# worxli/ORB_SLAM

Measured on AMD Instinct MI355X. Metric: frames/sec ORB extract+match (640x480, 1000 kp), higher is better.
Workload: dtype u8

## Files before the change

orb_slam_amd/csrc/orbx_device.h:

```cpp
#pragma once

#include <hip/hip_runtime.h>
#include <stdint.h>

#include "orbx_sincos.h"

namespace orbx {

#include "orbx_sincos_table.inc"

constexpr int kBlock = 256;
constexpr int kWaves = kBlock / 64;

__device__ inline float fast_atan2_deg(float y, float x)
{
    const float p1 = 0.9997878412794807f * (float)(180 / M_PI);
    const float p3 = -0.3258083974640975f * (float)(180 / M_PI);
    const float p5 = 0.1555786518463281f * (float)(180 / M_PI);
    const float p7 = -0.04432655554792128f * (float)(180 / M_PI);
    const float eps = (float)2.220446049250313e-16;
    const float ax = fabsf(x), ay = fabsf(y);
    float a;
    if (ax >= ay) {
        const float c = __fdiv_rn(ay, __fadd_rn(ax, eps));
// ... 356 lines not shown
            if (cl == m + 1) s.vars[0] = x;
            if (cl == 1) s.vars[2] = x;
        }
        if (k >= P) {
            if (cr <= m) posR[cr - 1] = x;
            if (cr == m) s.vars[1] = x;
            cr--;
        }
    }
    __syncthreads();
    for (int k = tid; k < m; k += kBlock) {
        const int i = posL[k], j = posR[k];
        const uint32_t t = a[i];
        a[i] = a[j];
        a[j] = t;
    }
    const int cut = (m == 0) ? s.vars[2] : min(s.vars[0], s.vars[1]);
    __syncthreads();
    return cut;
}

__device__ inline int floor_log2(int n)
{
    return 31 - __clz(n);
}

__device__ inline void block_nth_element(uint32_t* a, int n, int nth, int* pos, BlockScratch& s, int pivot_mode = 0)
{
    if (n == 0 || nth == n) return;
    int first = 0, last = n;
    int depth = 2 * floor_log2(n);
    while (last - first > 3) {
        if (depth == 0) {
            if (threadIdx.x == 0) {
                heap_select(a + first, nth + 1 - first, last - first);
                const uint32_t t = a[first];
                a[first] = a[nth];
                a[nth] = t;
            }
            __syncthreads();
            return;
        }
        --depth;
        if (threadIdx.x == 0) nth_pivot_step(a, first, last, pivot_mode);
        __syncthreads();
        const int cut = block_hoare_partition(a, first, last, pos, s);
        if (cut <= nth) first = cut;
        else last = cut;
    }
    if (threadIdx.x == 0) insertion_sort(a, first, last);
    __syncthreads();
}

__device__ inline void lds_wave_sync()
{
    __builtin_amdgcn_fence(__ATOMIC_RELEASE, "wavefront");
    __builtin_amdgcn_wave_barrier();
    __builtin_amdgcn_fence(__ATOMIC_ACQUIRE, "wavefront");
}

__device__ inline void global_wave_sync()
{
    __builtin_amdgcn_fence(__ATOMIC_RELEASE, "workgroup");
    __builtin_amdgcn_wave_barrier();
    __builtin_amdgcn_fence(__ATOMIC_ACQUIRE, "workgroup");
}

template <bool kGlobal>
__device__ inline void nth_sync()
{
    if constexpr (kGlobal) global_wave_sync();
    else lds_wave_sync();
}

__device__ inline int wave_min_int(int v)
{
#pragma unroll
    for (int o = 32; o > 0; o >>= 1) v = min(v, __shfl_xor(v, o, 64));
    return v;
}

template <bool kGlobal = false, typename E>
__device__ inline int wave_hoare_partition(E* a, int lo, int hi, int* pos)
{
    int* posR = pos;
    int* posL = pos + (hi - lo) / 2 + 1;
    const int lane = threadIdx.x & 63;
    const uint32_t P = kp_key(a[lo]);
    const int len = hi - lo - 1;
    const int chunk = (len + 63) / 64;
    const int s0 = min(lo + 1 + lane * chunk, hi), s1 = min(s0 + chunk, hi);
    int nle = 0, nge = 0;
    for (int x = s0; x < s1; x++) {
        const uint32_t k = kp_key(a[x]);
        nle += (k <= P);
        nge += (k >= P);
    }
    int le_incl, ge_incl;
    if (len < 65536) {
        const int both = wave_inclusive_scan(nle | (nge << 16));
        le_incl = both & 0xFFFF;
        ge_incl = (int)((uint32_t)both >> 16);
    } else {
        le_incl = wave_inclusive_scan(nle);
        ge_incl = wave_inclusive_scan(nge);
    }
    const int tot_ge = __builtin_amdgcn_readlane(ge_incl, 63);
    const int le_before = le_incl - nle;
    const int ge_after_chunk = tot_ge - ge_incl;
    int cl = le_before, cr = ge_after_chunk + nge, best = 0;
    for (int x = s0; x < s1; x++) {
        best = max(best, min(cl, cr));
        const uint32_t k = kp_key(a[x]);
        cl += (k <= P);
        cr -= (k >= P);
    }
    best = max(best, min(cl, cr));
    const int m = wave_max(best);
    int lm1 = 0x7fffffff, rm = -1, l1 = 0x7fffffff;
    cl = le_before;
    cr = ge_after_chunk + nge;
    for (int x = s0; x < s1; x++) {
        const uint32_t k = kp_key(a[x]);
        if (k <= P) {
            cl++;
            if (cl <= m) posL[cl - 1] = x;
            if (cl == m + 1) lm1 = x;
            if (cl == 1) l1 = x;
        }
        if (k >= P) {
            if (cr <= m) posR[cr - 1] = x;
            if (cr == m) rm = x;
            cr--;
        }
    }
    auto from_lane = [](int v, bool have, int none) {
        const unsigned long long b = __ballot(have);
        return b ? __builtin_amdgcn_readlane(v, (int)__builtin_ctzll(b)) : none;
    };
    lm1 = from_lane(lm1, lm1 != 0x7fffffff, 0x7fffffff);
    l1 = from_lane(l1, l1 != 0x7fffffff, 0x7fffffff);
    rm = from_lane(rm, rm >= 0, -1);
    nth_sync<kGlobal>();
    for (int k = lane; k < m; k += 64) {
        const int i = posL[k], j = posR[k];
        const E t = a[i];
        a[i] = a[j];
        a[j] = t;
    }
    nth_sync<kGlobal>();
    return (m == 0) ? l1 : min(lm1, rm);
}

template <bool kGlobal = false, typename E>
__device__ inline void wave_nth_element(E* a, int n, int nth, int* pos, int pivot_mode = 0)
{
    if (n == 0 || nth == n) return;
    const int lane = threadIdx.x & 63;
    int first = 0, last = n;
    int depth = 2 * floor_log2(n);
    while (last - first > 3) {
        if (depth == 0) {
            if (lane == 0) {
                heap_select(a + first, nth + 1 - first, last - first);
                const E t = a[first];
                a[first] = a[nth];
                a[nth] = t;
            }
            nth_sync<kGlobal>();
            return;
        }
        --depth;
        if (lane == 0) nth_pivot_step(a, first, last, pivot_mode);
        nth_sync<kGlobal>();
        const int cut = wave_hoare_partition<kGlobal>(a, first, last, pos);
        if (cut <= nth) first = cut;
        else last = cut;
    }
    if (lane == 0) insertion_sort(a, first, last);
    nth_sync<kGlobal>();
}

}
```

orb_slam_amd/csrc/orbx_extract.hip:

```cpp
#include <algorithm>
#include <type_traits>

#include "orbx_device.h"
#include "orbx_internal.h"

namespace orbx {

constexpr size_t kRetainLds = 128 * 1024;
constexpr int kRetainCellCap = 512;
constexpr int kSplitMinFrames = 16;
constexpr size_t kResizeLds = 96 * 1024;

__constant__ __attribute__((aligned(4))) int8_t c_pattern[256][4] = {
#include "orbx_pattern.inc"
};

#ifdef ORBX_FAST_PROFILE
__device__ unsigned long long g_fast_prof[24];
__device__ inline unsigned long long fp_stamp()
{
    unsigned long long t;
    asm volatile("s_memtime %0\n\ts_waitcnt lgkmcnt(0)" : "=s"(t)::"memory");
    return t;
}
// ... 1129 lines not shown
        tot[k] = 0;
        ret[k] = 0;
        nomore[k] = false;
        if (64 * k < nCells && c < nCells) {
            tot[k] = counts[c];
            if (a.cells[L.cell_base + c].valid) {
                if (tot[k] > nfc) {
                    ret[k] = nfc;
                } else {
                    ret[k] = tot[k];
                    toDist += nfc - tot[k];
                    nomore[k] = true;
                    nNoMore++;
                }
            }
        }
    }
    toDist = wave_sum(toDist);
    nNoMore = wave_sum(nNoMore);
    while (toDist > 0 && nNoMore < nCells) {
        const int nNew = nfc + (int)ceilf(__fdiv_rn((float)toDist, (float)(nCells - nNoMore)));
        int td = 0, nm = 0;
#pragma unroll
        for (int k = 0; k < kPer; k++) {
            if (64 * k >= nCells) break;
            const int c = lane + 64 * k;
            if (c < nCells && !nomore[k]) {
                if (tot[k] > nNew) {
                    ret[k] = nNew;
                } else {
                    ret[k] = tot[k];
                    td += nNew - tot[k];
                    nomore[k] = true;
                    nm++;
                }
            }
        }
        toDist = wave_sum(td);
        nNoMore += wave_sum(nm);
    }
    int base = 0, my_keep = 0, my_pre = 0;
#pragma unroll
    for (int k = 0; k < kPer; k++) {
        if (64 * k >= nCells) break;
        const int c = lane + 64 * k;
        const int take = (c < nCells && tot[k] > 0 && ret[k] > 0) ? min(tot[k], ret[k]) : 0;
        const int incl = wave_inclusive_scan(take);
        const int kk = __builtin_amdgcn_readlane(ret[k], cell & 63), pp = __builtin_amdgcn_readlane(base + incl - take, cell & 63);
        if ((cell >> 6) == k) {
            my_keep = kk;
            my_pre = pp;
        }
        base += __builtin_amdgcn_readlane(incl, 63);
    }
    *keep_c = my_keep;
    *pre_c = my_pre;
    *level_total = base;
}

constexpr float kHarrisK = 0.04f;
constexpr float kHarrisScale = 1.0f / ((1 << 2) * 7 * 255.0f);
constexpr float kHarrisScale4 = kHarrisScale * kHarrisScale * kHarrisScale * kHarrisScale;

__global__ __launch_bounds__(256) void k_harris_cells(ExtractArgs a)
{
    const int cell = blockIdx.x, f = blockIdx.y;
    const CellGeom C = cget(a.cells, cell);
    if (!C.valid) return;
    const int n = min(a.cell_count[(size_t)f * a.ncells + cell], C.list_cap);
    const LevelGeom L = cget(a.levels, C.level);
    const LevelSrc ls = level_src(a, f, C.level, L.off, L.stride);
    const int stride = ls.stride;
    const uint8_t* img = ls.base + (size_t)kEdge * stride + kEdge;
    const uint32_t* src = a.cell_lists + (size_t)f * a.list_entries + C.list_off;
    uint64_t* dst = a.cell_keys64 + (size_t)f * a.list_entries + C.list_off;
    for (int i = threadIdx.x; i < n; i += blockDim.x) {
        const uint32_t e = src[i];
        const int y = (int)((e >> 12) & 0xFFF), x = (int)(e & 0xFFF);
        const uint8_t* p0 = img + (ptrdiff_t)(y - 4) * stride + (x - 4);
        int r0[9], r1[9], r2[9];
#pragma unroll
        for (int j = 0; j < 9; j++) {
            r0[j] = p0[j];
            r1[j] = p0[stride + j];
        }
        int sa = 0, sb = 0, sc = 0;
#pragma unroll
        for (int rr = 2; rr < 9; rr++) {
#pragma unroll
            for (int j = 0; j < 9; j++) r2[j] = p0[(ptrdiff_t)rr * stride + j];
#pragma unroll
            for (int j = 1; j < 8; j++) {
                const int Ix = (r1[j + 1] - r1[j - 1]) * 2 + (r0[j + 1] - r0[j - 1]) + (r2[j + 1] - r2[j - 1]);
                const int Iy = (r2[j] - r0[j]) * 2 + (r2[j - 1] - r0[j - 1]) + (r2[j + 1] - r0[j + 1]);
                sa += Ix * Ix;
                sb += Iy * Iy;
                sc += Ix * Iy;
            }
#pragma unroll
            for (int j = 0; j < 9; j++) {
                r0[j] = r1[j];
                r1[j] = r2[j];
            }
        }
        const float fa = (float)sa, fb = (float)sb, fc = (float)sc;
        const float s2 = __fadd_rn(fa, fb);
        const float t = a.fp_contract
                            ? __fmaf_rn(-__fmul_rn(kHarrisK, s2), s2, __fmaf_rn(fa, fb, -__fmul_rn(fc, fc)))
                            : __fsub_rn(__fsub_rn(__fmul_rn(fa, fb), __fmul_rn(fc, fc)),
                                        __fmul_rn(__fmul_rn(kHarrisK, s2), s2));
        const float resp = __fmul_rn(t, kHarrisScale4);
        dst[i] = (uint64_t)harris_key(resp) << 32 | (e & 0xFFFFFFu);
    }
}

template <typename E>
__device__ inline E* cell_entries(const ExtractArgs& a)
{
    if constexpr (sizeof(E) == 8) return a.cell_keys64;
    else return a.cell_lists;
}
template <typename E>
__device__ inline E* level_entries(const ExtractArgs& a)
{
    if constexpr (sizeof(E) == 8) return a.level_keys64;
    else return a.level_keys;
}

template <typename E>
__global__ __launch_bounds__(256) void k_retain_cells(ExtractArgs a, int waves_per_block, int wave_words)
{
    extern __shared__ __attribute__((aligned(16))) uint32_t sbuf[];
    const int wv = threadIdx.x >> 6, lane = threadIdx.x & 63;
    const int cell = blockIdx.x * waves_per_block + wv, f = blockIdx.y;
    if (cell >= a.ncells) return;
    E* list = reinterpret_cast<E*>(sbuf + (size_t)wv * wave_words);
    int* pos = reinterpret_cast<int*>(list + kRetainCellCap);
    const CellGeom C = cget(a.cells, cell);
    const LevelGeom L = cget(a.levels, C.level);
    const int c = cell - L.cell_base;
    const int32_t* counts = a.cell_count + (size_t)f * a.ncells + L.cell_base;
    int k, pre, level_total;
    level_quota(a, L, counts, c, &k, &pre, &level_total);
    if (c == 0 && lane == 0) a.level_count[(size_t)f * a.nlevels + C.level] = min(level_total, L.level_cap);
    if (level_total > L.level_cap) {
        if (lane == 0) atomicOr(a.error_flags, 2);
        return;
    }
    const int n = counts[c];
    if (n == 0 || k == 0) return;
    const int take = min(n, k);
    E* src = cell_entries<E>(a) + (size_t)f * a.list_entries + C.list_off;
    E* dst = level_entries<E>(a) + (size_t)f * a.level_entries + L.level_off + pre;
    if (n > k && n <= kRetainCellCap) {
        stage_to_lds<8>(list, n, lane, 64, [&](int i) { return src[i]; });
        lds_wave_sync();
        wave_nth_element(list, n, k, pos, a.nth_pivot);
        for (int i = lane; i < take; i += 64) dst[i] = list[i];
    } else if (n > k) {
        int* gpos = a.retain_scratch + (size_t)f * (a.list_entries + 4 * a.ncells) + C.list_off + 4 * cell;
        wave_nth_element<true>(src, n, k, gpos, a.nth_pivot);
        for (int i = lane; i < take; i += 64) dst[i] = src[i];
    } else {
        for (int i = lane; i < take; i += 64) dst[i] = src[i];
    }
}

template <typename E>
__global__ __launch_bounds__(256) void k_retain_levels(ExtractArgs a, int waves_per_block, int wave_words)
{
    extern __shared__ __attribute__((aligned(16))) uint32_t sbuf[];
    const int wv = threadIdx.x >> 6, lane = threadIdx.x & 63;
    const int level = blockIdx.x * waves_per_block + wv, f = blockIdx.y;
    if (level >= a.nlevels) return;
    const LevelGeom L = cget(a.levels, level);
    int32_t* cnt = a.level_count + (size_t)f * a.nlevels + level;
    const int nlev = *cnt;
    if (nlev <= L.n_desired) return;
    E* list = reinterpret_cast<E*>(sbuf + (size_t)wv * wave_words);
    int* pos = reinterpret_cast<int*>(list + a.max_level_cap);
    E* g = level_entries<E>(a) + (size_t)f * a.level_entries + L.level_off;
    stage_to_lds<8>(list, nlev, lane, 64, [&](int i) { return g[i]; });
    lds_wave_sync();
    wave_nth_element(list, nlev, L.n_desired, pos, a.nth_pivot);
    for (int i = lane; i < L.n_desired; i += 64) g[i] = list[i];
    if (lane == 0) *cnt = L.n_desired;
}

typedef float orbx_f2 __attribute__((ext_vector_type(2)));

__device__ __forceinline__ void blur_hrow(uint32_t wl, uint32_t wc, uint32_t wr, orbx_f2 (&o)[2])
{
    int hs[4];
    blur_hsum_w(wl, wc, wr, hs);
    o[0] = orbx_f2{(float)hs[0], (float)hs[1]};
    o[1] = orbx_f2{(float)hs[2], (float)hs[3]};
}

__device__ __forceinline__ uint32_t blur_vstep(const orbx_f2 (&R)[7][2], uint32_t raw, const bool (&inside)[4],
                                               const bool (&tail_col)[4], bool any_tail)
{
    constexpr float kInv = 1.0f / 65536.0f;
    constexpr float k0 = 55.0f * kInv, k1 = 49.0f * kInv, k2 = 34.0f * kInv, k3 = 18.0f * kInv;
    float sv[4];
#pragma unroll
    for (int h = 0; h < 2; h++) {
        orbx_f2 N = R[3][h] * k0;
        N = __builtin_elementwise_fma(R[2][h] + R[4][h], orbx_f2{k1, k1}, N);
        N = __builtin_elementwise_fma(R[1][h] + R[5][h], orbx_f2{k2, k2}, N);
        N = __builtin_elementwise_fma(R[0][h] + R[6][h], orbx_f2{k3, k3}, N);
        sv[2 * h] = N.x;
        sv[2 * h + 1] = N.y;
        if (any_tail) {
            const orbx_f2 tl2 = N + 0.5f;
            if (tail_col[2 * h]) sv[2 * h] = floorf(tl2.x);
            if (tail_col[2 * h + 1]) sv[2 * h + 1] = floorf(tl2.y);
        }
    }
    uint32_t word = raw;
#pragma unroll
    for (int j = 0; j < 4; j++)
        if (inside[j]) word = __builtin_amdgcn_cvt_pk_u8_f32(sv[j], j, word);
    return word;
}

__device__ __forceinline__ void blur_block(const ExtractArgs& a, const int4* tiles, const int bx, const int f)
{
    const int4 tl = cget(tiles, bx);
    const int wi = tl.y + (threadIdx.x >> 6), lane = threadIdx.x & 63;
    if (wi >= tl.z * tl.w) return;
    const LevelGeom L = cget(a.levels, tl.x);
    const int strip = wi / tl.z, chunk = wi - strip * tl.z;
    const int ndw = L.stride >> 2;
    const int dw = kBlurChunkCols * chunk - 1 + lane;
    const bool out = lane >= 1 && lane <= kBlurChunkCols && dw < ndw;
    const int x = 4 * min(max(dw, 0), ndw - 1);
    const int y0 = strip * kBlurStrip, y1 = min(y0 + kBlurStrip, L.ph);
    const uint8_t* src = a.pyr_raw + (size_t)f * a.frame_pyr_bytes + L.off;
    uint8_t* dst = a.pyr_blur + (size_t)f * a.frame_pyr_bytes + L.off;
    const uint32_t stride = (uint32_t)L.stride;
    auto ld = [&](int y) { return *reinterpret_cast<const uint32_t*>(src + ((uint32_t)y * stride + (uint32_t)x)); };
    auto st = [&](int y, uint32_t v) {
        if (out) *reinterpret_cast<uint32_t*>(dst + ((uint32_t)y * stride + (uint32_t)x)) = v;
    };
    auto left = [&](uint32_t v) { return (uint32_t)__builtin_amdgcn_update_dpp(0, (int)v, 0x138, 0xf, 0xf, false); };
    auto right = [&](uint32_t v) { return (uint32_t)__builtin_amdgcn_update_dpp(0, (int)v, 0x130, 0xf, 0xf, false); };
    const int iy0 = kEdge, iy1 = kEdge + L.h;
    const int ya = min(max(y0, iy0), y1), yb = max(min(y1, iy1), ya);
    uint32_t keep_mask = 0;
#pragma unroll
    for (int j = 0; j < 4; j++)
        if (x + j < L.pw) keep_mask |= 0xFFu << (8 * j);
    auto copy_rows = [&](int ylo, int yhi) {
        for (int yc = ylo; yc < yhi; yc += 4) {
            uint32_t v[4];
#pragma unroll
            for (int k = 0; k < 4; k++) v[k] = ld(min(yc + k, yhi - 1));
#pragma unroll
            for (int k = 0; k < 4; k++)
                if (yc + k < yhi) st(yc + k, v[k] & keep_mask);
        }
    };
    copy_rows(y0, ya);
    if (ya < yb) {
        int half_even[4];
        bool inside[4];
#pragma unroll
        for (int j = 0; j < 4; j++) {
            const int xi = x + j - kEdge;
            inside[j] = xi >= 0 && xi < L.w;
            half_even[j] = xi < L.nvec_blur;
        }
        bool tail_col[4], any_tail = false;
#pragma unroll
        for (int j = 0; j < 4; j++) {
            tail_col[j] = inside[j] && !half_even[j];
            any_tail = any_tail || tail_col[j];
        }
        orbx_f2 R[7][2];
        auto hrow = [&](uint32_t c, orbx_f2 (&o)[2]) { blur_hrow(left(c), c, right(c), o); };
        uint32_t C[3];
        {
            uint32_t w0[6];
#pragma unroll
            for (int k = 0; k < 6; k++) w0[k] = ld(ya - 3 + k);
#pragma unroll
            for (int k = 0; k < 6; k++) {
                hrow(w0[k], R[k]);
                if (k >= 3) C[k - 3] = w0[k];
            }
        }
        constexpr int kBlurChunk = 7;
        for (int yc = ya; yc < yb; yc += kBlurChunk) {
            uint32_t wc[kBlurChunk];
#pragma unroll
            for (int k = 0; k < kBlurChunk; k++) wc[k] = ld(min(yc + k, yb - 1) + 3);
#pragma unroll
            for (int k = 0; k < kBlurChunk; k++) {
                const int y = yc + k;
                hrow(wc[k], R[6]);
                const uint32_t word = blur_vstep(R, C[0], inside, tail_col, any_tail);
                if (y < yb) st(y, word & keep_mask);
#pragma unroll
                for (int kk = 0; kk < 6; kk++)
#pragma unroll
                    for (int h = 0; h < 2; h++) R[kk][h] = R[kk + 1][h];
                C[0] = C[1];
// ... 201 lines not shown
};

template <bool kFma>
__global__ __launch_bounds__(256) __attribute__((amdgpu_waves_per_eu(5))) void k_describe(ExtractArgs a, int nframes)
{
    __shared__ __attribute__((aligned(16))) uint8_t s_patch[2 * kWaves][kDescWaveBytes];
    __shared__ int2 s_mom[2 * kWaves];
    __shared__ DescTrig s_trig[2 * kWaves];
    const XcdBlock xb = xcd_block();
    const int f = xb.frame, chunk = xb.chunk;
    if (f >= nframes) return;
    const int lane = threadIdx.x & 63, wv = __builtin_amdgcn_readfirstlane(threadIdx.x >> 6) & (kWaves - 1);
    const int half = lane >> 5, hl = lane & 31;
    const int slot = wv * 2 + half;
    const int k0 = chunk * (2 * kWaves) + wv * 2, k = k0 + half;
    const int umax_l = a.umax[min(lane, kHalfPatch)];
    uint32_t pat[8];
#pragma unroll
    for (int r = 0; r < 8; r++) pat[r] = *reinterpret_cast<const uint32_t*>(c_pattern[r * 32 + hl]);
    const int ll = min(lane, a.nlevels - 1);
    const int cnt_l = lane < a.nlevels ? a.level_count[(size_t)f * a.nlevels + lane] : 0;
    const long long off_l = a.levels[ll].off;
    const int stride_l = a.levels[ll].stride, loff_l = a.levels[ll].level_off;
    const int w_l = a.levels[ll].w, h_l = a.levels[ll].h, nvec_l = a.levels[ll].nvec_blur;
    const float scale_l = a.levels[ll].scale, psize_l = a.levels[ll].patch_size;
    int total = 0, level0 = -1, local0 = 0, level1 = -1, local1 = 0;
    for (int l = 0; l < a.nlevels; l++) {
        const int c = __builtin_amdgcn_readlane(cnt_l, l);
        if (level0 < 0 && k0 < total + c) {
            level0 = l;
            local0 = k0 - total;
        }
        if (level1 < 0 && k0 + 1 < total + c) {
            level1 = l;
            local1 = k0 + 1 - total;
        }
        total += c;
    }
    int level = half ? level1 : level0, local = half ? local1 : local0;
    if (k == 0 && lane == 0) {
        a.out_n[a.first_slot + f] = total;
        if (a.host_out) {
            reinterpret_cast<int32_t*>(a.host_out)[0] = total;
            reinterpret_cast<int32_t*>(a.host_out)[1] = *a.error_flags;
        }
    }
    if (chunk * (2 * kWaves) >= total) return;
    const bool valid = level >= 0;
    const bool wave_on = level0 >= 0;
    if (!valid) {
        level = 0;
        local = 0;
    }
    int x = 0, y = 0, X = 0, Y = 0, lev_w = 0, lev_h = 0, lev_nvec = 0;
    float lev_scale = 0.f, lev_psize = 0.f, response = 0.f;
    uint8_t* win = s_patch[slot] + kWinPad;
    const uint8_t* br = win;
    int m01 = 0, m10 = 0;
    if (wave_on) {
        auto pick = [&](int v) { return __builtin_amdgcn_ds_bpermute(level << 2, v); };
        const long long lev_off = (long long)(((unsigned long long)(uint32_t)pick((int)(off_l >> 32)) << 32) |
                                              (uint32_t)pick((int)off_l));
        const int lev_stride = pick(stride_l), lev_loff = pick(loff_l);
        lev_w = pick(w_l);
        lev_h = pick(h_l);
        lev_nvec = pick(nvec_l);
        lev_scale = __int_as_float(pick(__float_as_int(scale_l)));
        lev_psize = __int_as_float(pick(__float_as_int(psize_l)));
        uint32_t e;
        if (a.harris) {
            const uint64_t e64 = a.level_keys64[(size_t)f * a.level_entries + lev_loff + local];
            e = (uint32_t)e64;
            response = harris_response((uint32_t)(e64 >> 32));
        } else {
            e = a.level_keys[(size_t)f * a.level_entries + lev_loff + local];
            response = (float)(e >> 24);
        }
        y = (int)((e >> 12) & 0xFFF);
        x = (int)(e & 0xFFF);
        X = kEdge + (valid ? x : kHalfPatch + 8);
        Y = kEdge + (valid ? y : kHalfPatch + 8);
        const LevelSrc ls = level_src(a, f, level, lev_off, lev_stride);
        const uint8_t* ic = win + describe_stage_window(ls.base, (uint32_t)ls.stride, a.l0_direct && level == 0, lev_w,
                                                        lev_h, X, Y, win, hl);
        br = ic;
        wave_lds_sync();
        if (hl < kIcRows) {
            const int u = hl - kHalfPatch;
            m10 = u * ic[u];
#pragma unroll
            for (int v = 1; v <= kHalfPatch; v++) {
                const int d = __builtin_amdgcn_readlane(umax_l, v);
                if (u >= -d && u <= d) {
                    const int vp = ic[u + v * kBrPitch], vm = ic[u - v * kBrPitch];
                    m01 += v * (vp - vm);
                    m10 += u * (vp + vm);
                }
            }
        }
        m01 = half_wave_sum(m01);
        m10 = half_wave_sum(m10);
    }
    if (hl == 0) s_mom[slot] = int2{m01, m10};
    __syncthreads();
    if (wv == ((chunk + f) & (kWaves - 1)) && lane < 2 * kWaves) {
        const int2 m = s_mom[lane];
        const float ang = fast_atan2_deg((float)m.x, (float)m.y);
        const float factorPI = (float)(M_PI / 180.f);
        float s, c;
        cr_sincosf(__fmul_rn(ang, factorPI), &s, &c);
        s_trig[lane] = DescTrig{ang, s, c};
    }
    if (wave_on) describe_blur_window(win, X, Y, lev_w, lev_h, lev_nvec, hl);
    __syncthreads();
    if (!wave_on) return;
    const float angle = s_trig[slot].angle, sa = s_trig[slot].sa, ca = s_trig[slot].ca;
    uint8_t* desc = a.out_desc + ((size_t)(a.first_slot + f) * a.nfeatures + k) * 32;
    const uint8_t* lds_bytes = &s_patch[0][0];
    const float brf = (float)(int)(br - lds_bytes);
#pragma unroll
    for (int r = 0; r < 8; r++) {
        const orbx_f2 px = {(float)(int8_t)(pat[r] & 0xFF), (float)(int8_t)((pat[r] >> 16) & 0xFF)};
        const orbx_f2 py = {(float)(int8_t)((pat[r] >> 8) & 0xFF), (float)(int8_t)(pat[r] >> 24)};
        uint32_t a1, a2;
        orb_sample_addr2<kFma>(px, py, sa, ca, brf, a1, a2);
        const int t0 = lds_bytes[a1];
        const int t1 = lds_bytes[a2];
        const unsigned long long bits = __ballot(t0 < t1);
        if (valid && hl == r) {
            reinterpret_cast<uint32_t*>(desc)[r] = (uint32_t)(bits >> (32 * half));
            if (a.host_out)
                reinterpret_cast<uint32_t*>(a.host_out + 64 + (size_t)a.nfeatures * sizeof(orbx_keypoint) +
                                            (size_t)k * 32)[r] = (uint32_t)(bits >> (32 * half));
        }
    }
    if (valid && hl == 0) {
        orbx_keypoint kp;
        kp.x = (float)x;
        kp.y = (float)y;
        if (level != 0) {
            kp.x = __fmul_rn(kp.x, lev_scale);
            kp.y = __fmul_rn(kp.y, lev_scale);
        }
        kp.size = lev_psize;
        kp.angle = angle;
        kp.response = response;
        kp.octave = level;
        kp.class_id = -1;
        a.out_kps[(size_t)(a.first_slot + f) * a.nfeatures + k] = kp;
        if (a.host_out) reinterpret_cast<orbx_keypoint*>(a.host_out + 64)[k] = kp;
    }
}

__global__ __launch_bounds__(64) void k_debug_nth(const uint32_t* in, int n, int nth, uint32_t* out_glb,
                                                  uint32_t* out_lds, int* gpos, int pivot_mode)
{
    __shared__ uint32_t list[kRetainCellCap];
    __shared__ int pos[kRetainCellCap + 8];
    const int lane = threadIdx.x;
    for (int i = lane; i < n; i += 64) out_glb[i] = in[i];
    global_wave_sync();
    wave_nth_element<true>(out_glb, n, nth, gpos, pivot_mode);
    for (int i = lane; i < n; i += 64) list[i] = in[i];
    lds_wave_sync();
    wave_nth_element(list, n, nth, pos, pivot_mode);
    for (int i = lane; i < n; i += 64) out_lds[i] = list[i];
}

}

extern "C" int orbx_debug_nth_pivot(const uint32_t* entries, int n, int nth, int pivot_mode, uint32_t* out_glb,
                                    uint32_t* out_lds)
{
    using namespace orbx;
    if (!entries || !out_glb || !out_lds || n < 0 || n > kRetainCellCap || nth < 0 || nth > n ||
        (pivot_mode != 0 && pivot_mode != 1))
        return ORBX_ERR_ARG;
    uint32_t* d = nullptr;
    if (hipMalloc(&d, 4 * sizeof(uint32_t) * (n + 8)) != hipSuccess) return ORBX_ERR_NOMEM;
    int r = ORBX_OK;
    if (hipMemcpy(d, entries, sizeof(uint32_t) * n, hipMemcpyHostToDevice) != hipSuccess) r = ORBX_ERR_HIP;
    if (r == ORBX_OK) {
        hipLaunchKernelGGL(k_debug_nth, dim3(1), dim3(64), 0, 0, d, n, nth, d + (n + 8), d + 2 * (n + 8),
                           reinterpret_cast<int*>(d + 3 * (n + 8)), pivot_mode);
        if (hipDeviceSynchronize() != hipSuccess ||
            hipMemcpy(out_glb, d + (n + 8), sizeof(uint32_t) * n, hipMemcpyDeviceToHost) != hipSuccess ||
            hipMemcpy(out_lds, d + 2 * (n + 8), sizeof(uint32_t) * n, hipMemcpyDeviceToHost) != hipSuccess)
            r = ORBX_ERR_HIP;
    }
    (void)hipFree(d);
    return r;
}

extern "C" int orbx_debug_nth(const uint32_t* entries, int n, int nth, uint32_t* out_glb, uint32_t* out_lds)
{
    return orbx_debug_nth_pivot(entries, n, nth, ORBX_NTH_PIVOT_GCC48, out_glb, out_lds);
}

namespace orbx {

__global__ __launch_bounds__(64) void k_debug_describe_patch(const uint8_t* lev, int stride, int direct, LevelGeom L,
                                                             int X, int Y, uint8_t* out)
{
    __shared__ __attribute__((aligned(16))) uint8_t s_patch[2][kDescWaveBytes];
    const int lane = threadIdx.x, half = lane >> 5, hl = lane & 31;
    uint8_t* win = s_patch[half] + kWinPad;
    const int centre = describe_stage_window(lev, (uint32_t)stride, direct != 0, L.w, L.h, X, Y, win, hl);
    wave_lds_sync();
    describe_blur_window(win, X, Y, L.w, L.h, L.nvec_blur, hl);
    if (half == 0)
        for (int i = hl; i < kBrRows * kBrRows; i += 32) {
            const int r = i / kBrRows, c = i - r * kBrRows;
            out[i] = win[centre + (r - kBrR) * kBrPitch + (c - kBrR)];
        }
}

static void launch_level0(const Geometry& g, const ExtractArgs& x, int nb, hipStream_t st)
{
    const LevelGeom& L = g.levels[0];
    const int qpr = L.stride / 16;
    int q_lo = (kEdge + 15) / 16, q_hi = (L.w + kEdge + kPyr0Shift - 32) / 16;
    q_hi = std::min(q_hi, qpr - 1);
    const int nint = (g.w % 16 == 0 && q_hi >= q_lo) ? q_hi - q_lo + 1 : 0;
    if (nint == 0) q_lo = 0;
    const int items = nint * ((L.ph + kPyrRows - 1) / kPyrRows) + (qpr - nint) * L.ph;
    hipLaunchKernelGGL(k_pyr_level0, dim3((items + 255) / 256, nb), dim3(256), 0, st, x, q_lo, nint);
}

int launch_level0_slot(orbx_ctx* ctx, int slot)
{
    ExtractArgs a = {};
    a.levels = ctx->dgeom.levels;
    a.frames = ctx->frames;
    a.first_slot = slot;
    a.pyr_raw = ctx->pyr_raw + (size_t)slot * ctx->geom.frame_pyr_bytes;
    a.frame_pyr_bytes = ctx->geom.frame_pyr_bytes;
    a.w = ctx->geom.w;
    a.h = ctx->geom.h;
    launch_level0(ctx->geom, a, 1, ctx->stream);
    if (hipGetLastError() != hipSuccess) return ORBX_ERR_HIP;
    return ORBX_OK;
}

int launch_blur_slot(orbx_ctx* ctx, int slot)
{
    const int r0 = launch_level0_slot(ctx, slot);
    if (r0 != ORBX_OK) return r0;
    ExtractArgs a = {};
    a.levels = ctx->dgeom.levels;
    a.pyr_raw = ctx->pyr_raw + (size_t)slot * ctx->geom.frame_pyr_bytes;
    a.pyr_blur = ctx->pyr_blur;
    a.frame_pyr_bytes = ctx->geom.frame_pyr_bytes;
    hipLaunchKernelGGL(k_blur, dim3(ctx->blur_tiles_n, 1), dim3(kBlurItems), 0, ctx->stream, a, ctx->blur_tiles);
    if (hipGetLastError() != hipSuccess) return ORBX_ERR_HIP;
    return ORBX_OK;
}

}

extern "C" int orbx_debug_describe_patch(orbx_ctx* ctx, int slot, int level, int x, int y, uint8_t* out)
{
    using namespace orbx;
    if (!ctx || !out || slot < 0 || slot >= ctx->slots || level < 0 || level >= ctx->geom.nlevels) return ORBX_ERR_ARG;
    const LevelGeom& L = ctx->geom.levels[level];
    if (x < kEdge || x >= L.w - kEdge || y < kEdge || y >= L.h - kEdge) return ORBX_ERR_ARG;
    ctx_enter(ctx);
    uint8_t* d = nullptr;
    if (hipDeviceSynchronize() != hipSuccess) return ORBX_ERR_HIP;
    if (hipMalloc(&d, kBrRows * kBrRows) != hipSuccess) return ORBX_ERR_NOMEM;
    const bool direct = level == 0 && kEdge == 16 && ctx->geom.w % 16 == 0;
    const long long fw = ctx->geom.w, fh = ctx->geom.h;
    const uint8_t* lev = direct ? ctx->frames + ((long long)slot * fw * fh - (long long)kEdge * fw - kEdge)
                                : ctx->pyr_raw + (size_t)slot * ctx->geom.frame_pyr_bytes + L.off;
    hipLaunchKernelGGL(k_debug_describe_patch, dim3(1), dim3(64), 0, ctx->stream, lev, direct ? (int)fw : L.stride,
                       direct ? 1 : 0, L, kEdge + x, kEdge + y, d);
    int r = ORBX_OK;
    if (hipStreamSynchronize(ctx->stream) != hipSuccess ||
        hipMemcpy(out, d, kBrRows * kBrRows, hipMemcpyDeviceToHost) != hipSuccess)
        r = ORBX_ERR_HIP;
    (void)hipFree(d);
    return r;
}

extern "C" int orbx_debug_level0_direct(orbx_ctx* ctx)
{
    if (!ctx) return ORBX_ERR_ARG;
    return ctx->last_l0_direct ? 1 : 0;
}

extern "C" int orbx_debug_fast_instance(orbx_ctx* ctx, int* out)
{
    if (!ctx || !out || ctx->last_fast[0] < 0) return ORBX_ERR_ARG;
    for (int k = 0; k < 3; k++) out[k] = ctx->last_fast[k];
    return ORBX_OK;
}

extern "C" int orbx_debug_fast_lists(orbx_ctx* ctx, int slot, int32_t* cells, int cells_cap, uint32_t* lists,
                                     int lists_cap, int* entries)
{
    using namespace orbx;
    if (!ctx || !cells || !lists || !entries || slot < 0 || slot >= ctx->slots) return ORBX_ERR_ARG;
    ctx_enter(ctx);
    const Geometry& g = ctx->geom;
    const int n = (int)g.cells.size();
    if (cells_cap < 10 * n || lists_cap < g.list_entries) return ORBX_ERR_CAPACITY;
    std::vector<int32_t> cnt(n);
    if (hipDeviceSynchronize() != hipSuccess ||
        hipMemcpy(cnt.data(), ctx->cell_count + (size_t)slot * n, 4 * (size_t)n, hipMemcpyDeviceToHost) != hipSuccess ||
        hipMemcpy(lists, ctx->cell_lists + (size_t)slot * g.list_entries, 4 * (size_t)g.list_entries,
                  hipMemcpyDeviceToHost) != hipSuccess)
        return ORBX_ERR_HIP;
    for (int c = 0; c < n; c++) {
        const CellGeom& C = g.cells[c];
        const int32_t v[10] = {C.level, C.ini_x, C.ini_y, C.hx, C.hy, C.valid ? 1 : 0, C.list_off, C.list_cap, cnt[c], 0};
        for (int k = 0; k < 10; k++) cells[10 * c + k] = v[k];
    }
    *entries = g.list_entries;
    return n;
}

namespace orbx {

int launch_extract(orbx_ctx* ctx, int first, int count, const MatchSpec* m)
{
    const Geometry& g = ctx->geom;
    if (count > 1 || (m && m->kind != 0 && ctx->async_match)) {
        const int r = ensure_aux_streams(ctx);
        if (r != ORBX_OK) return r;
    }
    for (int sl = first; sl < first + count && sl < (int)ctx->bow_ready.size(); sl++) ctx->bow_ready[sl] = 0;
    wait_uploads_overlap(ctx, first, count, ctx->stream);
    ExtractArgs a;
    a.levels = ctx->dgeom.levels;
    a.cells = ctx->dgeom.cells;
    a.res_cols = ctx->dgeom.res_cols;
    a.res_rows = ctx->dgeom.res_rows;
    a.umax = ctx->dgeom.umax;
    a.frames = ctx->frames;
    a.pyr_raw = ctx->pyr_raw + (size_t)first * g.frame_pyr_bytes;
    a.pyr_blur = nullptr;
    a.cell_lists = ctx->cell_lists + (size_t)first * g.list_entries;
    a.cell_count = ctx->cell_count + (size_t)first * g.cells.size();
    a.level_keys = ctx->level_keys + (size_t)first * g.level_entries;
    a.level_count = ctx->level_count + (size_t)first * g.nlevels;
// ... 289 lines not shown
```

Before: 304,000.

## Do small nth_element partitions in wave registers instead of LDS

Adds a register-resident introselect that holds each element in one lane and partitions with ballots, mbcnt and ds_permute/bpermute, with no LDS round trips or serial lane-0 steps. Cells with at most 64 candidates now skip LDS staging entirely. Larger selections fall through to the register path once the range shrinks to 64, replacing the serial lane-0 insertion sort. The debug entry points are templated over 64-bit entries for testing. The risk is that the result must match the old selection order exactly for parity, and the extra cross-lane traffic per round.

```diff
diff --git a/orb_slam_amd/csrc/orbx_device.h b/orb_slam_amd/csrc/orbx_device.h
--- a/orb_slam_amd/csrc/orbx_device.h
+++ b/orb_slam_amd/csrc/orbx_device.h
@@ -532,33 +532,168 @@
     return (m == 0) ? l1 : min(lm1, rm);
 }
 
+__device__ inline uint32_t lane_get(uint32_t v, int i) { return __builtin_amdgcn_readlane(v, i); }
+__device__ inline uint64_t lane_get(uint64_t v, int i)
+{
+    return (uint64_t)(uint32_t)__builtin_amdgcn_readlane((uint32_t)(v >> 32), i) << 32 |
+           (uint32_t)__builtin_amdgcn_readlane((uint32_t)v, i);
+}
+template <typename E>
+__device__ inline E lane_set(E v, E s, int i) { return (int)(threadIdx.x & 63) == i ? s : v; }
+__device__ inline uint32_t lane_pull(uint32_t v, int src) { return __builtin_amdgcn_ds_bpermute(src << 2, v); }
+__device__ inline uint64_t lane_pull(uint64_t v, int src)
+{
+    return (uint64_t)(uint32_t)__builtin_amdgcn_ds_bpermute(src << 2, (uint32_t)(v >> 32)) << 32 |
+           (uint32_t)__builtin_amdgcn_ds_bpermute(src << 2, (uint32_t)v);
+}
+__device__ inline int lane_rank(unsigned long long m)
+{
+    return __builtin_amdgcn_mbcnt_hi((uint32_t)(m >> 32), __builtin_amdgcn_mbcnt_lo((uint32_t)m, 0));
+}
+
+template <typename E>
+__device__ inline bool wave_nth_rounds_reg(E& v, int& first_io, int& last_io, int& depth_io, int nth, int pivot_mode)
+{
+    const int lane = threadIdx.x & 63;
+    int first = __builtin_amdgcn_readfirstlane(first_io), last = __builtin_amdgcn_readfirstlane(last_io);
+    int depth = __builtin_amdgcn_readfirstlane(depth_io);
+    nth = __builtin_amdgcn_readfirstlane(nth);
+    bool done = true;
+    while (last - first > 3) {
+        if (depth == 0) {
+            done = false;
+            break;
+        }
+        --depth;
+        {
+            const uint32_t key = kp_key(v);
+            const int x = pivot_mode == 1 ? first : first + 1, y = first + (last - first) / 2, z = last - 1;
+            const uint32_t kx = __builtin_amdgcn_readlane(key, x), ky = __builtin_amdgcn_readlane(key, y),
+                           kz = __builtin_amdgcn_readlane(key, z);
+            int t;
+            if (kx > ky) t = ky > kz ? y : (kx > kz ? z : x);
+            else t = kx > kz ? x : (ky > kz ? z : y);
+            if (t != first) {
+                const E ef = lane_get(v, first), et = lane_get(v, t);
+                v = lane_set(v, et, first);
+                v = lane_set(v, ef, t);
+            }
+        }
+        const uint32_t key = kp_key(v);
+        const uint32_t P = __builtin_amdgcn_readlane(key, first);
+        const bool inr = (unsigned)(lane - first - 1) < (unsigned)(last - first - 1);
+        const bool is_le = inr && key <= P, is_ge = inr && key >= P;
+        const unsigned long long le = __ballot(is_le), ge = __ballot(is_ge);
+        const int n_le = __builtin_popcountll(le);
+        const int cl = lane_rank(le);
+        const int cr = __builtin_popcountll(ge) - lane_rank(ge);
+        const unsigned long long cross = __ballot(cl >= cr) & ~((2ull << first) - 1);
+        const int sx = cross ? (int)__builtin_ctzll(cross) : 64;
+        const int m = max(sx < 64 ? __builtin_amdgcn_readlane(cr, sx) : 0, __builtin_amdgcn_readlane(cl, sx - 1));
+        const int posL = __builtin_amdgcn_ds_permute((is_le ? cl : 63) << 2, lane);
+        const int posR = __builtin_amdgcn_ds_permute((is_ge ? cr - 1 : 63) << 2, lane);
+        const bool isL = is_le && cl < m, isR = is_ge && cr <= m;
+        const int pk = __builtin_amdgcn_ds_bpermute((isL ? cl : cr - 1) << 2, posL | (posR << 8));
+        const int partner = isL ? (pk >> 8) & 0xff : (isR ? pk & 0xff : lane);
+        v = lane_pull(v, partner);
+        int cut;
+        if (m == 0) {
+            cut = le ? (int)__builtin_ctzll(le) : last;
+        } else {
+            const int lm1 = m < n_le ? __builtin_amdgcn_readlane(posL, m) : 0x7fffffff;
+            cut = min(lm1, __builtin_amdgcn_readlane(posR, m - 1));
+        }
+        if (cut <= nth) first = cut;
+        else last = cut;
+    }
+    if (done && last - first >= 2) {
+        E e0 = lane_get(v, first), e1 = lane_get(v, first + 1);
+        if (kp_greater(e1, e0)) {
+            const E t = e0;
+            e0 = e1;
+            e1 = t;
+        }
+        if (last - first == 3) {
+            E e2 = lane_get(v, first + 2);
+            if (kp_greater(e2, e0)) {
+                const E t = e2;
+                e2 = e1;
+                e1 = e0;
+                e0 = t;
+            } else if (kp_greater(e2, e1)) {
+                const E t = e2;
+                e2 = e1;
+                e1 = t;
+            }
+            v = lane_set(v, e2, first + 2);
+        }
+        v = lane_set(v, e0, first);
+        v = lane_set(v, e1, first + 1);
+    }
+    first_io = first;
+    last_io = last;
+    depth_io = depth;
+    return done;
+}
+
+template <bool kGlobal, typename E>
+__device__ inline void wave_nth_heap_fallback(E* a, int first, int last, int nth)
+{
+    if ((threadIdx.x & 63) == 0) {
+        heap_select(a + first, nth + 1 - first, last - first);
+        const E t = a[first];
+        a[first] = a[nth];
+        a[nth] = t;
+    }
+    nth_sync<kGlobal>();
+}
+
 template <bool kGlobal = false, typename E>
 __device__ inline void wave_nth_element(E* a, int n, int nth, int* pos, int pivot_mode = 0)
 {
+    n = __builtin_amdgcn_readfirstlane(n);
+    nth = __builtin_amdgcn_readfirstlane(nth);
     if (n == 0 || nth == n) return;
     const int lane = threadIdx.x & 63;
     int first = 0, last = n;
     int depth = 2 * floor_log2(n);
-    while (last - first > 3) {
+    while (last - first > 64) {
         if (depth == 0) {
-            if (lane == 0) {
-                heap_select(a + first, nth + 1 - first, last - first);
-                const E t = a[first];
-                a[first] = a[nth];
-                a[nth] = t;
-            }
-            nth_sync<kGlobal>();
+            wave_nth_heap_fallback<kGlobal>(a, first, last, nth);
             return;
         }
         --depth;
         if (lane == 0) nth_pivot_step(a, first, last, pivot_mode);
         nth_sync<kGlobal>();
-        const int cut = wave_hoare_partition<kGlobal>(a, first, last, pos);
+        const int cut = __builtin_amdgcn_readfirstlane(wave_hoare_partition<kGlobal>(a, first, last, pos));
         if (cut <= nth) first = cut;
         else last = cut;
     }
-    if (lane == 0) insertion_sort(a, first, last);
+    const int base = first, cnt = last - first;
+    E v = lane < cnt ? a[base + lane] : E(0);
+    int f = 0, l = cnt;
+    const bool done = wave_nth_rounds_reg(v, f, l, depth, nth - base, pivot_mode);
+    if (lane < cnt) a[base + lane] = v;
     nth_sync<kGlobal>();
-}
-
-}
+    if (!done) wave_nth_heap_fallback<kGlobal>(a, base + f, base + l, nth);
+}
+
+template <typename E>
+__device__ inline E wave_nth_element_small(E v, int n, int nth, E* spill, int pivot_mode = 0)
+{
+    n = __builtin_amdgcn_readfirstlane(n);
+    nth = __builtin_amdgcn_readfirstlane(nth);
+    if (n == 0 || nth == n) return v;
+    const int lane = threadIdx.x & 63;
+    int f = 0, l = n;
+    int depth = 2 * floor_log2(n);
+    if (!wave_nth_rounds_reg(v, f, l, depth, nth, pivot_mode)) {
+        if (lane < n) spill[lane] = v;
+        lds_wave_sync();
+        wave_nth_heap_fallback<false>(spill, f, l, nth);
+        if (lane < n) v = spill[lane];
+    }
+    return v;
+}
+
+}
diff --git a/orb_slam_amd/csrc/orbx_extract.hip b/orb_slam_amd/csrc/orbx_extract.hip
--- a/orb_slam_amd/csrc/orbx_extract.hip
+++ b/orb_slam_amd/csrc/orbx_extract.hip
@@ -1305,7 +1305,10 @@
     const int take = min(n, k);
     E* src = cell_entries<E>(a) + (size_t)f * a.list_entries + C.list_off;
     E* dst = level_entries<E>(a) + (size_t)f * a.level_entries + L.level_off + pre;
-    if (n > k && n <= kRetainCellCap) {
+    if (n > k && n <= 64) {
+        const E v = wave_nth_element_small(lane < n ? src[lane] : E(0), n, k, list, a.nth_pivot);
+        if (lane < take) dst[lane] = v;
+    } else if (n > k && n <= kRetainCellCap) {
         stage_to_lds<8>(list, n, lane, 64, [&](int i) { return src[i]; });
         lds_wave_sync();
         wave_nth_element(list, n, k, pos, a.nth_pivot);
@@ -1813,10 +1816,11 @@
     }
 }
 
-__global__ __launch_bounds__(64) void k_debug_nth(const uint32_t* in, int n, int nth, uint32_t* out_glb,
-                                                  uint32_t* out_lds, int* gpos, int pivot_mode)
-{
-    __shared__ uint32_t list[kRetainCellCap];
+template <typename E>
+__global__ __launch_bounds__(64) void k_debug_nth(const E* in, int n, int nth, E* out_glb, E* out_lds, int* gpos,
+                                                  int pivot_mode)
+{
+    __shared__ E list[kRetainCellCap];
     __shared__ int pos[kRetainCellCap + 8];
     const int lane = threadIdx.x;
     for (int i = lane; i < n; i += 64) out_glb[i] = in[i];
@@ -1828,29 +1832,44 @@
     for (int i = lane; i < n; i += 64) out_lds[i] = list[i];
 }
 
-}
-
-extern "C" int orbx_debug_nth_pivot(const uint32_t* entries, int n, int nth, int pivot_mode, uint32_t* out_glb,
-                                    uint32_t* out_lds)
-{
-    using namespace orbx;
+template <typename E>
+int debug_nth(const E* entries, int n, int nth, int pivot_mode, E* out_glb, E* out_lds)
+{
     if (!entries || !out_glb || !out_lds || n < 0 || n > kRetainCellCap || nth < 0 || nth > n ||
         (pivot_mode != 0 && pivot_mode != 1))
         return ORBX_ERR_ARG;
-    uint32_t* d = nullptr;
-    if (hipMalloc(&d, 4 * sizeof(uint32_t) * (n + 8)) != hipSuccess) return ORBX_ERR_NOMEM;
+    E* d = nullptr;
+    if (hipMalloc(&d, 4 * sizeof(E) * (n + 8)) != hipSuccess) return ORBX_ERR_NOMEM;
     int r = ORBX_OK;
-    if (hipMemcpy(d, entries, sizeof(uint32_t) * n, hipMemcpyHostToDevice) != hipSuccess) r = ORBX_ERR_HIP;
+    if (hipMemcpy(d, entries, sizeof(E) * n, hipMemcpyHostToDevice) != hipSuccess) r = ORBX_ERR_HIP;
     if (r == ORBX_OK) {
-        hipLaunchKernelGGL(k_debug_nth, dim3(1), dim3(64), 0, 0, d, n, nth, d + (n + 8), d + 2 * (n + 8),
+        hipLaunchKernelGGL(k_debug_nth<E>, dim3(1), dim3(64), 0, 0, d, n, nth, d + (n + 8), d + 2 * (n + 8),
                            reinterpret_cast<int*>(d + 3 * (n + 8)), pivot_mode);
         if (hipDeviceSynchronize() != hipSuccess ||
-            hipMemcpy(out_glb, d + (n + 8), sizeof(uint32_t) * n, hipMemcpyDeviceToHost) != hipSuccess ||
-            hipMemcpy(out_lds, d + 2 * (n + 8), sizeof(uint32_t) * n, hipMemcpyDeviceToHost) != hipSuccess)
+            hipMemcpy(out_glb, d + (n + 8), sizeof(E) * n, hipMemcpyDeviceToHost) != hipSuccess ||
+            hipMemcpy(out_lds, d + 2 * (n + 8), sizeof(E) * n, hipMemcpyDeviceToHost) != hipSuccess)
             r = ORBX_ERR_HIP;
     }
     (void)hipFree(d);
     return r;
+}
+
+}
+
+extern "C" int orbx_debug_nth_pivot(const uint32_t* entries, int n, int nth, int pivot_mode, uint32_t* out_glb,
+                                    uint32_t* out_lds)
+{
+    return orbx::debug_nth(entries, n, nth, pivot_mode, out_glb, out_lds);
+}
+
+extern "C" int orbx_debug_nth64(const float* responses, int n, int nth, int pivot_mode, uint64_t* out_glb,
+                                uint64_t* out_lds)
+{
+    if (!responses || n < 0 || n > orbx::kRetainCellCap) return ORBX_ERR_ARG;
+    std::vector<uint64_t> e((size_t)n);
+    for (int i = 0; i < n; i++) e[i] = (uint64_t)orbx::harris_key(responses[i]) << 32 | (uint32_t)i;
+    static const uint64_t none = 0;
+    return orbx::debug_nth(n ? e.data() : &none, n, nth, pivot_mode, out_glb, out_lds);
 }
 
 extern "C" int orbx_debug_nth(const uint32_t* entries, int n, int nth, uint32_t* out_glb, uint32_t* out_lds)
```

Result: faster. 311,200, median of 6 (+2.4%).
